# gasparian/CRNN-OCR-lite

Hardware: AMD Instinct MI355X
Metric: text-line images/sec (train step) (higher is better)
Workload: dtype bf16; 1 GPU; BASELINE configs[1]: 100x32x1 text lines, batch 256/GPU, max_len 23, time_dense_size 128, n_units 256 BiLSTM, STN on, dropout on, CTC, Adam(1e-4,b1=.5,clipnorm 5), bf16 MFMA products, bf16 conv-stack tensors in HBM, fp32 accumulate/statistics/RNN/optimizer (outside the 1e-3 parity tolerance: see parity_mode for the fp32 step); global_batch=256, parallelism=dp1, parity_mode_backward_planes=2 (16 significant bits per factor; CRNN_FLAG_THREE_PLANE_BACKWARD = strict)

## Files before the change

crnn-ocr-lite_amd/crnn_mi355x/native.py:

```python
import ctypes
import os
import re
import subprocess

HERE = os.path.dirname(os.path.abspath(__file__))
PKG_ROOT = os.path.dirname(HERE)
REPO_ROOT = os.path.dirname(PKG_ROOT)
HEADER = os.path.join(REPO_ROOT, "include", "crnn_mi355x.h")
CSRC = os.path.join(PKG_ROOT, "csrc")
LIB_PATH = os.path.join(PKG_ROOT, "libcrnn_mi355x.so")
HOOKS_HEADER = os.path.join(REPO_ROOT, "include", "crnn_testhooks.h")
HOOKS_PATH = os.path.join(PKG_ROOT, "libcrnn_testhooks.so")
SOURCES = ["gemm.hip", "gemm_nt.hip", "gemm_wres.hip", "gemm_wres3.hip", "gemm_wgrad.hip", "gemm_wgrad3.hip", "gemm_pres.hip", "conv.hip", "conv_bwd_fused.hip", "dwconv_stream.hip", "dwconv_bwd_stream.hip", "stn.hip", "rnn.hip", "rnn_persist.hip", "gru_persist.hip", "ctc.hip", "dense.hip", "beam.hip", "score.hip", "optim.hip", "ingest.hip", "model.hip"]


class crnn_config(ctypes.Structure):
    _fields_ = [(n, ctypes.c_int) for n in
                ("batch", "imgh", "imgw", "num_classes", "max_len", "tds", "units", "gru", "stn", "dropout", "mfma_bf16", "flags")]


FLAG_RNN_STEP_KERNELS = 1
FLAG_GEMM_TILE_KERNELS = 2
FLAG_NO_DW_BN_FUSION = 8
FLAG_NO_DW_BWD_FUSION = 16
FLAG_DW_TILE_KERNEL = 32
FLAG_RNN_LINEAR_CLUSTERS = 64
FLAG_NO_BN_STATS_FUSION = 128
FLAG_F32_MFMA_GEMMS = 256
FLAG_BN2_DW_FUSION = 1024
FLAG_BN2_STATS_FUSION = 2048
FLAG_BLOCK1_KERNELS = 16384
FLAG_LOC_NET_KERNELS = 8192
FLAG_THREE_PLANE_BACKWARD = 65536
FLAG_TWO_PLANE_FORWARD = 131072
FLAG_NO_GRADIENT_PLANES = 262144
FLAG_NO_POOL_ARGMAX_Q = 524288
FLAG_NO_BN2_DW_FUSION = 4096
RNN_XCD_LOCAL = 0x100


_CTYPE = [("crnn_stream_t", ctypes.c_void_p), ("size_t", ctypes.c_size_t), ("uint64_t", ctypes.c_uint64),
          ("uint32_t", ctypes.c_uint32), ("long", ctypes.c_long), ("int", ctypes.c_int), ("float", ctypes.c_float),
          ("double", ctypes.c_double)]


def _ctype_of(decl):
    decl = decl.strip()
    if "*" in decl:
        return ctypes.c_void_p
    for key, ct in _CTYPE:
        if re.search(r"\b%s\b" % key, decl):
# ... 91 lines not shown
```

crnn-ocr-lite_amd/csrc/conv.hip:

```cpp
#include "common.h"
#include <stdlib.h>

#define BN_EPS 1e-3f
#ifndef DW_NT
#define DW_NT 256
#endif

template <int VEC>
struct VecF { float v[VEC]; };

#ifndef CRNN_NT_BN_BWD2
#define CRNN_NT_BN_BWD2 1
#endif
#ifndef CRNN_NT_BN_ACT
#define CRNN_NT_BN_ACT 1
#endif
template <int VEC, typename T>
__device__ __forceinline__ VecF<VEC> vload_nt(const T* p);
template <int VEC, bool NT, typename T>
__device__ __forceinline__ VecF<VEC> vload_s(const T* p);
template <int VEC, typename T>
__device__ __forceinline__ VecF<VEC> vload(const T* p) {
  VecF<VEC> r;
  if (VEC == 8) {
// ... 2 lines not shown
    r.v[4 % VEC] = q.hi.x; r.v[5 % VEC] = q.hi.y; r.v[6 % VEC] = q.hi.z; r.v[7 % VEC] = q.hi.w;
  } else if (VEC == 4) {
    float4 q = ld4(p); r.v[0] = q.x; r.v[1 % VEC] = q.y; r.v[2 % VEC] = q.z; r.v[3 % VEC] = q.w;
  } else {
    r.v[0] = ld1(p);
  }
  return r;
}
template <int VEC, typename T>
__device__ __forceinline__ void vstore(T* p, const VecF<VEC>& r) {
  if (VEC == 8) {
    float8 q;
    q.lo = make_float4(r.v[0], r.v[1 % VEC], r.v[2 % VEC], r.v[3 % VEC]);
    q.hi = make_float4(r.v[4 % VEC], r.v[5 % VEC], r.v[6 % VEC], r.v[7 % VEC]);
    st8(p, q);
  } else if (VEC == 4) {
    st4(p, make_float4(r.v[0], r.v[1 % VEC], r.v[2 % VEC], r.v[3 % VEC]));
  } else {
    st1(p, r.v[0]);
  }
}
template <typename T> struct VecMax { static const int value = 4; };
template <> struct VecMax<bf16_t> { static const int value = 8; };

#ifndef DW_BF16_VN
#define DW_BF16_VN 4
#endif
template <typename T> struct RawV;
template <> struct RawV<float> { typedef float4 type; static const int N = 4; };
#if DW_BF16_VN == 8
template <> struct RawV<bf16_t> { typedef uint4 type; static const int N = 8; };
#else
template <> struct RawV<bf16_t> { typedef uint2 type; static const int N = 4; };
#endif
template <typename V, typename T> __device__ __forceinline__ V ldraw(const T* p) { return *reinterpret_cast<const V*>(p); }
__device__ __forceinline__ void widen(const float4& v, float (&f)[4]) { f[0] = v.x; f[1] = v.y; f[2] = v.z; f[3] = v.w; }
__device__ __forceinline__ void widen(const uint2& u, float (&f)[4]) {
  f[0] = __uint_as_float(u.x << 16); f[1] = __uint_as_float(u.x & 0xffff0000u);
  f[2] = __uint_as_float(u.y << 16); f[3] = __uint_as_float(u.y & 0xffff0000u);
}
__device__ __forceinline__ void widen(const uint4& u, float (&f)[8]) {
  f[0] = __uint_as_float(u.x << 16); f[1] = __uint_as_float(u.x & 0xffff0000u);
  f[2] = __uint_as_float(u.y << 16); f[3] = __uint_as_float(u.y & 0xffff0000u);
  f[4] = __uint_as_float(u.z << 16); f[5] = __uint_as_float(u.z & 0xffff0000u);
  f[6] = __uint_as_float(u.w << 16); f[7] = __uint_as_float(u.w & 0xffff0000u);
}
// ... 696 lines not shown
  if (dt_in == CRNN_BF16) return bn_act_launch((const bf16_t*)x, bnstate, (float*)y, B, H, W, C, ph, pw, rate, seed, layer, stream);
  if (dt_out == CRNN_BF16) return bn_act_launch((const float*)x, bnstate, (bf16_t*)y, B, H, W, C, ph, pw, rate, seed, layer, stream);
  return bn_act_launch((const float*)x, bnstate, (float*)y, B, H, W, C, ph, pw, rate, seed, layer, stream);
}
extern "C" int crnn_bn_act_pool_drop_qmax_ex(const void* x, const float* bnstate, void* y, void* qmax, int B, int H, int W, int C, int ph, int pw, float rate,
                                             uint64_t seed, uint32_t layer, int dt_in, int dt_out, hipStream_t stream) {
  if (!x || !bnstate || !qmax) return CRNN_ERR_ARG;
  if (dt_in == CRNN_BF16 && dt_out == CRNN_BF16) return bn_act_launch((const bf16_t*)x, bnstate, (bf16_t*)y, B, H, W, C, ph, pw, rate, seed, layer, stream, (bf16_t*)qmax);
  if (dt_in == CRNN_BF16) return bn_act_launch((const bf16_t*)x, bnstate, (float*)y, B, H, W, C, ph, pw, rate, seed, layer, stream, (bf16_t*)qmax);
  if (dt_out == CRNN_BF16) return bn_act_launch((const float*)x, bnstate, (bf16_t*)y, B, H, W, C, ph, pw, rate, seed, layer, stream, (float*)qmax);
  return bn_act_launch((const float*)x, bnstate, (float*)y, B, H, W, C, ph, pw, rate, seed, layer, stream, (float*)qmax);
}
extern "C" int crnn_bn_act_pool_drop(const float* x, const float* bnstate, float* y, int B, int H, int W, int C, int ph,
                                     int pw, float rate, uint64_t seed, uint32_t layer, hipStream_t stream) {
  return crnn_bn_act_pool_drop_ex(x, bnstate, y, B, H, W, C, ph, pw, rate, seed, layer, CRNN_F32, CRNN_F32, stream);
}

template <typename T>
struct BnBwdArgsT {
  const T* x; const T* g; const float* bnstate; const float* gamma;
  int B, H, W, C, ph, pw; float rate; uint64_t seed; uint32_t layer;
  unsigned short* dxp = nullptr; long dxps = 0; int dxpl = 0;
  const T* qmax = nullptr;
};
template <int VEC, typename T>
__device__ __forceinline__ void bn_store_dx(const BnBwdArgsT<T>& a, T* dx, long idx, const VecF<VEC>& o) {
  if constexpr (VEC == 4 && sizeof(T) == 4) {
    if (a.dxp) {
      unsigned w0[3], w1[3];
      crnn_split3_pair(o.v[0], o.v[1], w0[0], w0[1], w0[2]);
      crnn_split3_pair(o.v[2 % VEC], o.v[3 % VEC], w1[0], w1[1], w1[2]);
      unsigned short* q = a.dxp + idx;
      *reinterpret_cast<uint2*>(q) = make_uint2(w0[0], w1[0]);
      *reinterpret_cast<uint2*>(q + a.dxps) = make_uint2(w0[1], w1[1]);
      if (a.dxpl == 3) *reinterpret_cast<uint2*>(q + 2 * a.dxps) = make_uint2(w0[2], w1[2]);
      return;
    }
  }
  vstore<VEC>(&dx[idx], o);
}

template <int VEC, typename T>
__device__ __forceinline__ VecF<VEC> vload_nt(const T* p) {
  typedef unsigned u32x4_nt __attribute__((ext_vector_type(4)));
  VecF<VEC> r;
  if constexpr (VEC == 8 && sizeof(T) == 2) {
    const u32x4_nt u = __builtin_nontemporal_load(reinterpret_cast<const u32x4_nt*>(p));
// ... 42 lines not shown
      for (int j = 0; j < a.pw; ++j) {
        if (ii == si && j == sj) continue;
        VecF<VEC> o = vload_s<VEC, NT>(&a.x[(((long)b * a.H + ho * a.ph + ii) * a.W + wo * a.pw + j) * a.C + c0]);
        bool earlier = (ii < si) || (ii == si && j < sj);
#pragma unroll
        for (int e = 0; e < VEC; ++e) {
          float oy = relu6f(fmaf(o.v[e], sc.v[e], sh.v[e]));
          if (earlier ? (oy >= y.v[e]) : (oy > y.v[e])) arg[e] = false;
        }
      }
    oidx = (((long)b * Ho + ho) * Wo + wo) * a.C + c0;
  }
  VecF<VEC> gv = vload_s<VEC, NT>(&a.g[oidx]);
  float dm[VEC];
  drop_scale_vec<VEC>(a.seed, a.layer, (uint64_t)oidx, a.rate, inv_keep, dm);
#pragma unroll
  for (int e = 0; e < VEC; ++e) {
    bool live = arg[e] && (y.v[e] > 0.f) && (y.v[e] < 6.f);
    out.v[e] = live ? gv.v[e] * dm[e] : 0.f;
  }
  return out;
}

template <int PASS, int VEC, bool POOL, typename T>
__global__ __launch_bounds__(256) void bn_bwd_kernel(BnBwdArgsT<T> a, float* __restrict__ partials,
                                                     const float* __restrict__ coef, T* __restrict__ dx, int CW,
                                                     int rows_per_chunk) {
  __shared__ float red[2][256 * VEC];
  const int tid = threadIdx.x, cl = tid % CW, rt = tid / CW, RT = 256 / CW;
  const long M = (long)a.B * a.H * a.W;
  const long r0 = (long)blockIdx.x * rows_per_chunk;
  long r1 = r0 + rows_per_chunk; if (r1 > M) r1 = M;
  const int CL = a.C / VEC;
  const float inv_keep = a.rate > 0.f ? 1.f / (1.f - a.rate) : 1.f;
  for (int cb = 0; cb < CL; cb += CW) {
    const int c = cb + cl, c0 = c * VEC;
    VecF<VEC> s, q;
#pragma unroll
    for (int e = 0; e < VEC; ++e) { s.v[e] = 0.f; q.v[e] = 0.f; }
    if (c < CL) {
      VecF<VEC> mu = vload<VEC>(a.bnstate + c0), var = vload<VEC>(a.bnstate + a.C + c0);
      VecF<VEC> sc = vload<VEC>(a.bnstate + 2 * a.C + c0), sh = vload<VEC>(a.bnstate + 3 * a.C + c0);
      VecF<VEC> inv, c1, c2;
#pragma unroll
      for (int e = 0; e < VEC; ++e) { inv.v[e] = 1.0f / sqrtf(var.v[e] + BN_EPS); c1.v[e] = 0.f; c2.v[e] = 0.f; }
      VecF<VEC> Pc, Qc;
#pragma unroll
      for (int e = 0; e < VEC; ++e) { Pc.v[e] = 0.f; Qc.v[e] = 0.f; }
      if (PASS == 2) {
        c1 = vload<VEC>(coef + c0); c2 = vload<VEC>(coef + a.C + c0);
#pragma unroll
        for (int e = 0; e < VEC; ++e) bn_bwd_pq(sc.v[e], c1.v[e], c2.v[e], mu.v[e], inv.v[e], Pc.v[e], Qc.v[e]);
      }
      long r = r0 + rt;
#if CRNN_BNB_ROWS4
      if (PASS == 1 && !POOL) {
        for (; r + 3L * RT < r1; r += 4L * RT) {
          VecF<VEC> xr[4], gr[4];
#pragma unroll
          for (int u = 0; u < 4; ++u) xr[u] = vload<VEC>(&a.x[(r + u * RT) * a.C + c0]);
#pragma unroll
          for (int u = 0; u < 4; ++u) gr[u] = bn_gy_vec<VEC, POOL, T>(a, r + u * RT, c0, xr[u], sc, sh, inv_keep);
#pragma unroll
          for (int u = 0; u < 4; ++u)
#pragma unroll
            for (int e = 0; e < VEC; ++e) { s.v[e] += gr[u].v[e]; q.v[e] = fmaf(gr[u].v[e], (xr[u].v[e] - mu.v[e]) * inv.v[e], q.v[e]); }
        }
      }
#endif
      constexpr bool NT = CRNN_NT_BN_BWD2 && PASS == 2;
      for (; r + RT < r1; r += 2L * RT) {
        VecF<VEC> xa = vload_s<VEC, NT>(&a.x[r * a.C + c0]);
        VecF<VEC> xb = vload_s<VEC, NT>(&a.x[(r + RT) * a.C + c0]);
        VecF<VEC> ga = bn_gy_vec<VEC, POOL, T, NT>(a, r, c0, xa, sc, sh, inv_keep);
        VecF<VEC> gb = bn_gy_vec<VEC, POOL, T, NT>(a, r + RT, c0, xb, sc, sh, inv_keep);
        VecF<VEC> oa, ob;
#pragma unroll
        for (int e = 0; e < VEC; ++e) {
          float ha = (xa.v[e] - mu.v[e]) * inv.v[e], hb = (xb.v[e] - mu.v[e]) * inv.v[e];
          if (PASS == 1) {
            s.v[e] += ga.v[e]; q.v[e] = fmaf(ga.v[e], ha, q.v[e]);
            s.v[e] += gb.v[e]; q.v[e] = fmaf(gb.v[e], hb, q.v[e]);
          } else {
            oa.v[e] = bn_bwd_dx_pq(xa.v[e], ga.v[e], sc.v[e], Pc.v[e], Qc.v[e]);
            ob.v[e] = bn_bwd_dx_pq(xb.v[e], gb.v[e], sc.v[e], Pc.v[e], Qc.v[e]);
          }
        }
        if (PASS == 2) { bn_store_dx<VEC, T>(a, dx, r * a.C + c0, oa); bn_store_dx<VEC, T>(a, dx, (r + RT) * a.C + c0, ob); }
      }
      for (; r < r1; r += RT) {
        VecF<VEC> xv = vload_s<VEC, NT>(&a.x[r * a.C + c0]);
        VecF<VEC> gy = bn_gy_vec<VEC, POOL, T, NT>(a, r, c0, xv, sc, sh, inv_keep);
        VecF<VEC> o;
#pragma unroll
        for (int e = 0; e < VEC; ++e) {
          float xh = (xv.v[e] - mu.v[e]) * inv.v[e];
          if (PASS == 1) { s.v[e] += gy.v[e]; q.v[e] = fmaf(gy.v[e], xh, q.v[e]); }
          else o.v[e] = bn_bwd_dx_pq(xv.v[e], gy.v[e], sc.v[e], Pc.v[e], Qc.v[e]);
        }
        if (PASS == 2) bn_store_dx<VEC, T>(a, dx, r * a.C + c0, o);
      }
    }
    if (PASS == 1) {
      __syncthreads();
#pragma unroll
      for (int e = 0; e < VEC; ++e) { red[0][tid * VEC + e] = s.v[e]; red[1][tid * VEC + e] = q.v[e]; }
      __syncthreads();
      if (rt == 0 && c < CL) {
#pragma unroll
        for (int e = 0; e < VEC; ++e) {
          float s2 = 0.f, q2 = 0.f;
          for (int r = 0; r < RT; ++r) { s2 += red[0][(r * CW + cl) * VEC + e]; q2 += red[1][(r * CW + cl) * VEC + e]; }
          partials[((long)blockIdx.x * 2 + 0) * a.C + c0 + e] = s2;
          partials[((long)blockIdx.x * 2 + 1) * a.C + c0 + e] = q2;
// ... 771 lines not shown
  return CRNN_OK;
}
extern "C" int crnn_dwconv_c1_bwd_rows(int B, int H, int W) { return cdiv((long)B * H * W, 1024); }
extern "C" int crnn_dwconv3x3_c1_bwd(const float* d, const float* da, const float* bnstate, const float* coef, const float* x, const float* k, float* dx, float* dk,
                                     float* scratch, int B, int H, int W, hipStream_t stream) {
  if (!d || !da || !bnstate || !coef || !x || !k || !dk || !scratch || B <= 0 || H <= 0 || W <= 0) return CRNN_ERR_ARG;
  if ((long)B * H * W >= (1L << 31) || W > C1B_MAXW) return CRNN_ERR_UNSUPPORTED;
  const int rows = crnn_dwconv_c1_bwd_rows(B, H, W);
  hipLaunchKernelGGL(dwconv_c1_bwd_kernel, dim3(rows), dim3(256), 0, stream, d, da, bnstate, coef, x, k, dx, scratch, B, H, W);
  CRNN_LAUNCH_CHECK();
  return crnn_partials_sum(scratch, rows, 9, dk, 1.f, stream);
}
extern "C" int crnn_pw1_bn_bwd_rows(long M) { return cdiv(M, colreduce_rpc(M)); }
extern "C" int crnn_pw1_bn_bwd(const float* d, const float* in_bnstate, const float* w, const void* dq, float* da, float* dw, float* scratch,
                               float* bn_stat_partials, long M, int N, int dt_q, hipStream_t stream) {
  if (!d || !in_bnstate || !w || !dq || !da || !dw || !scratch || !bn_stat_partials) return CRNN_ERR_ARG;
  if (!pw1_ok(N, dq) || M <= 0 || N < 8) return CRNN_ERR_UNSUPPORTED;
  const int rpc = colreduce_rpc(M), chunks = cdiv(M, rpc);
  if (dt_q == CRNN_BF16) hipLaunchKernelGGL(pw1_bn_bwd_kernel<bf16_t>, dim3(chunks), dim3(256), 0, stream, d, in_bnstate, w, (const bf16_t*)dq, da, scratch, bn_stat_partials, M, N, rpc);
  else hipLaunchKernelGGL(pw1_bn_bwd_kernel<float>, dim3(chunks), dim3(256), 0, stream, d, in_bnstate, w, (const float*)dq, da, scratch, bn_stat_partials, M, N, rpc);
  CRNN_LAUNCH_CHECK();
  return crnn_partials_sum(scratch, chunks, N, dw, 1.f, stream);
}
```

crnn-ocr-lite_amd/csrc/model.hip:

```cpp
#include "common.h"
#include "crnn_mi355x.h"
#include <string.h>
#include <stdio.h>
#include <string>
#include <vector>

namespace {

struct BlockSpec { int cout, ph, pw; };
const BlockSpec kBlocks[7] = {{64, 1, 1}, {128, 1, 1}, {256, 2, 2}, {256, 1, 1}, {512, 1, 2}, {512, 1, 1}, {512, 1, 1}};
bool pool_argmax_q(const crnn_config* cfg, int block) {
  const int ph = kBlocks[block - 1].ph, pw = kBlocks[block - 1].pw;
  return !(cfg->flags & CRNN_FLAG_NO_POOL_ARGMAX_Q) && ((ph == 2 && pw == 2) || (ph == 1 && pw == 2));
}
const float kDropBlock = 0.1f, kDropDense1 = 0.4f, kDropRnn = 0.2f;
const uint32_t kLayerDense1 = 8, kLayerRnn = 9;

struct Tensor { std::string name; long off; long size; int ndim; int dims[4]; int dtype = CRNN_F32; };

struct Dims {
  int B, H0, W0, Hp, Wp, T, feat, C, L, tds, u, G, stn_flat;
  int Hs1, Ws1, Ho1, Wo1, Hs2, Ws2, Ho2, Wo2;
  int bh[8], bw[8], bc[8];
};
// ... 275 lines not shown
  return ((((uintptr_t)a) | ((uintptr_t)b) | ((uintptr_t)c) | ((uintptr_t)d)) & 15) == 0;
}
bool fuse_bn2_dw_shape(const crnn_config* cfg, const Dims& d, const Plan& P, int i) {
  if (i < 1 || i > 6) return false;
  if (!bn2_dw_fusion_block(cfg, i) || (cfg->flags & (CRNN_FLAG_DW_TILE_KERNEL | CRNN_FLAG_NO_DW_BWD_FUSION))) return false;
  const std::string p = std::to_string(i), n = std::to_string(i + 1);
  const bool pooled = kBlocks[i - 1].ph * kBlocks[i - 1].pw != 1;
  if (pooled && (!pool_argmax_q(cfg, i) || !P.has("qm" + p) || d.bh[i] % kBlocks[i - 1].ph || d.bw[i] % kBlocks[i - 1].pw || d.bc[i] % 4 ||
                 (long)d.B * d.bh[i + 1] * d.bw[i + 1] * d.bc[i] + 8192L * 256 * 8 >= (1L << 31))) return false;
  const int dt = P.dt("q" + p);
  if (P.dt("x" + p) != dt || P.dt("d" + n) != dt || P.off("dm" + p) < 0) return false;
  if (bn2_stats_fusion_block(cfg, i) && P.off("bn2parts") < 0) return false;
  const int H = d.bh[i + 1], W = d.bw[i + 1], C = d.bc[i];
  return crnn_dwconv_fwd_stream_pro_supported_ex(d.B, H, W, C, dt) == CRNN_OK && crnn_dwconv_bwd_stream_pro_supported_ex(d.B, H, W, C, dt) == CRNN_OK &&
         (dt == CRNN_F32 || crnn_dwconv_bwd_fused_supported(H, W, C) == CRNN_OK);
}
float* pro_src(const Ctx& c, int i) { return c.w((kBlocks[i - 1].ph * kBlocks[i - 1].pw != 1 ? "qm" : "q") + std::to_string(i)); }
bool fuse_bn2_dw(const Ctx& c, int i) {
  if (!fuse_bn2_dw_shape(c.cfg, c.d, c.P, i)) return false;
  const std::string p = std::to_string(i), n = std::to_string(i + 1);
  return aligned16(c.w("q" + p), c.w("bn2s" + p), c.w("d" + n), c.p("b" + n + "_dw")) && aligned16(pro_src(c, i));
}
const float* keep_bytes(const Ctx& c, int i) { return c.cfg->dropout ? c.w("dm" + std::to_string(i)) : nullptr; }
int gemm32(const Ctx& c, int mode, const float* A, const float* B, float* C, int M, int N, int K, int lda, int ldb, int ldc,
           const float* bias = nullptr, int act = 0, int acc = 0, int perm = 0) {
  return crnn_gemm_f32(mode, A, B, C, M, N, K, lda, ldb, ldc, bias, act, acc, perm, c.scratch(), kGemmScratchBytes, c.s);
}

int colsum(const Ctx& c, const float* x, long M, int C, int ld, float* out) {
  CRNN_TRY(crnn_colreduce(x, c.partials(), M, C, ld, 1, c.s));
  return crnn_partials_sum(c.partials(), crnn_colreduce_chunks(M), C, out, 1.f, c.s);
}

int check_cfg(const crnn_config* c) {
  if (!c || c->batch <= 0) return CRNN_ERR_ARG;
  if (c->units < 64 || c->units % 64) return CRNN_ERR_UNSUPPORTED;
  if (c->mfma_bf16 < 0 || c->mfma_bf16 > 2) return CRNN_ERR_ARG;
  if (c->num_classes > 64 || c->num_classes < 2) return CRNN_ERR_UNSUPPORTED;
  if (2 * c->max_len + 1 > 64) return CRNN_ERR_UNSUPPORTED;
  if (c->tds % 4) return CRNN_ERR_UNSUPPORTED;
  Dims d = make_dims(c);
  if (c->stn && (d.Ho2 < 1 || d.Wo2 < 1)) return CRNN_ERR_UNSUPPORTED;
  if (d.T < 3 || d.feat < 1) return CRNN_ERR_UNSUPPORTED;
  return 0;
}

// ... 280 lines not shown
          rc = conv_planes(cfg, false) == 2 ? crnn_pwconv_bnrelu6_fwd_f32x2(dd, s1, c.p(bp + "_pw"), qq, M, co, ci, parts, stream)
                                            : crnn_pwconv_bnrelu6_fwd_f32x3(dd, s1, c.p(bp + "_pw"), qq, M, co, ci, parts, stream);
        CRNN_TRY(rc);
      }
      else if (fuse_a) {
        int rc = CRNN_ERR_UNSUPPORTED;
        if (wt && dtq == CRNN_BF16 && !(cfg->flags & CRNN_FLAG_GEMM_TILE_KERNELS) && crnn_pwconv_fwd_wres_supported(M, co, ci) == CRNN_OK) {
          rc = crnn_pwconv_bnrelu6_fwd_wres(dd, s1, wq, qq, M, co, ci, parts, stream);
          if (rc == CRNN_OK) stat_rows = crnn_pwconv_fwd_wres_rows(M, co, ci);
        }
        if (rc == CRNN_ERR_UNSUPPORTED) rc = crnn_pwconv_bnrelu6_fwd(dd, s1, wq, qq, M, co, ci, parts, dtq, wt, stream);
        CRNN_TRY(rc);
      } else CRNN_TRY(crnn_pwconv_fwd(aa, wq, qq, M, co, ci, parts, nullptr, pw_products_fwd(cfg),
                                      dtd, dtw, dtq, wt, stream));
    }
    CRNN_TRY(crnn_bn_finalize_folded(parts, stat_rows, co, M, c.p(bp + "_bn2_g"), c.p(bp + "_bn2_b"), s2, c.w("fold"), stream));
    bn_off += co;
    if (fuse_bn2_dw(c, i)) {
      if (ph * pw != 1)
        CRNN_TRY(crnn_bn_act_pool_drop_qmax_ex(qq, s2, nullptr, pro_src(c, i), B, H, W, co, ph, pw, 0.f, seed, (uint32_t)i, dtq, dtq, stream));
      pro_q = pro_src(c, i); pro_s2 = s2; in = nullptr;
      continue;
    }
    if (use_qmax(c, i))
      CRNN_TRY(crnn_bn_act_pool_drop_qmax_ex(qq, s2, xo, c.w("qm" + p), B, H, W, co, ph, pw, cfg->dropout ? kDropBlock : 0.f, seed, (uint32_t)i, dtq, c.dt("x" + p), stream));
    else
    CRNN_TRY(crnn_bn_act_pool_drop_ex(qq, s2, xo, B, H, W, co, ph, pw, cfg->dropout ? kDropBlock : 0.f, seed,
                                      (uint32_t)i, dtq, c.dt("x" + p), stream));
    in = xo;
  }
  if (keep_pending) { CRNN_TRY(fj.join()); keep_pending = false; }
  const int T = d.T, TB = T * B, u = d.u, G = d.G;
  int rc1 = CRNN_ERR_UNSUPPORTED;
  if (d1T_off >= 0 && c.dt("x7") == CRNN_BF16)
    rc1 = crnn_dense_fwd_stream(in, reinterpret_cast<const bf16_t*>(c.w("pwT")) + d1T_off, c.p("dense1_b"), c.w("dn1"), TB, d.tds, d.feat, d.feat, d.feat, 1, T,
                                (train && cfg->dropout) ? kDropDense1 : 0.f, seed, kLayerDense1, stream);
  if (rc1 != CRNN_OK && rc1 != CRNN_ERR_UNSUPPORTED) return rc1;
  if (rc1 != CRNN_OK) {
    CRNN_TRY(gemm_t(c, 0, in, c.dt("x7"), c.p("dense1_w"), CRNN_F32, c.w("dn1"), CRNN_F32, TB, d.tds, d.feat, d.feat, d.tds, d.tds, c.p("dense1_b"), 1, 0, T));
    if (train && cfg->dropout) CRNN_TRY(crnn_dropout(c.w("dn1"), c.w("dn1"), TB, d.tds, d.tds, d.tds, kDropDense1, seed, kLayerDense1, stream));
  }
  const int dtu = rnn_dtu(cfg);
  const bool persist = rnn_persist(cfg);
  const size_t xbytes = persist ? crnn_lstm_persist_xbuf_bytes(T, B, u, dtu) : 0;
  const bool xw_stream = dtu == CRNN_BF16 && !(cfg->flags & CRNN_FLAG_GEMM_TILE_KERNELS) && TB % 64 == 0 && G % 128 == 0 && d.tds % 64 == 0 && u % 64 == 0;
  {
    long in_off[8], out_off[8]; int R[8], Cc[8]; int n = 0;
// ... 292 lines not shown
  float* gA = c.w("gA"); float* gB = c.w("gB"); float* gC = c.w("gC");
  hipEvent_t gB_free = nullptr, gC_free = nullptr;
  int bn2_stats_rows = 0;
  for (int i = 7; i >= 1; --i) {
    std::string p = std::to_string(i), bp = "b" + p;
    const int H = d.bh[i], W = d.bw[i], ci = d.bc[i - 1], co = d.bc[i];
    const long M = (long)B * H * W;
    const int dtd = c.dt("d" + p), dtq = c.dt("q" + p);
    const bool fused_bf = i > 1 && dtd == CRNN_BF16 && c.dt("x" + std::to_string(i - 1)) == CRNN_BF16 && !(cfg->flags & CRNN_FLAG_NO_DW_BWD_FUSION) &&
                          crnn_dwconv_bwd_fused_supported(H, W, ci) == CRNN_OK;
    const bool fused_f32 = i > 1 && dtd == CRNN_F32 && dtq == CRNN_F32 && c.dt("x" + std::to_string(i - 1)) == CRNN_F32 &&
                           !(cfg->flags & (CRNN_FLAG_NO_DW_BWD_FUSION | CRNN_FLAG_DW_TILE_KERNEL)) &&
                           crnn_dwconv_bwd_stream_supported_ex(B, H, W, ci, CRNN_F32) == CRNN_OK &&
                           aligned16(c.w("d" + p), c.w("x" + std::to_string(i - 1)), c.p(bp + "_dw"), c.w("coef")) && aligned16(gA, gB, gC, c.w("bn1s" + p));
    const bool fused_dw = fused_bf || fused_f32;
    int bn1_stats_rows = 0;
    const bool dq_planes = !fused_bf && pw_products(cfg) == 2 && conv_planes(cfg, true) == 2 && dtq == CRNN_F32 && dtd == CRNN_F32 && fuse_dw_bn_x3(cfg, dtd, dtq, ci) &&
                           !(cfg->flags & (CRNN_FLAG_GEMM_TILE_KERNELS | CRNN_FLAG_NO_BN_STATS_FUSION | CRNN_FLAG_NO_GRADIENT_PLANES)) &&
                           (kBlocks[i - 1].ph * kBlocks[i - 1].pw == 1 || crnn_knob("CRNN_DQPL_POOL", 1)) &&
                           crnn_gemm_pres_supported(M, ci, co, 2) == CRNN_OK && crnn_pwconv_wgrad_planes_stream_supported(M, co, ci) == CRNN_OK &&
                           crnn_pwconv_wgrad_planes_stream_scratch_bytes(M, co, ci) <= kGemmScratchBytes &&
                           aligned16(c.w("d" + p), c.w("q" + p), c.w("bn1s" + p), c.p(bp + "_pw")) && aligned16(gA, gB, gC, c.w("partials"));
    CRNN_TRY(fj.wait(gB_free)); gB_free = nullptr;
    if (bn2_stats_rows > 0) {
      CRNN_TRY(crnn_bn_bwd_finalize(c.w("bn2parts"), bn2_stats_rows, co, M, c.g(bp + "_bn2_g"), c.g(bp + "_bn2_b"), c.w("coef"), stream));
      if (dq_planes)
        CRNN_TRY(crnn_bn_bwd_apply_planes_ex(c.w("q" + p), gA, c.w("bn2s" + p), c.w("coef"), gB, M * co, 2, B, H, W, co, kBlocks[i - 1].ph, kBlocks[i - 1].pw,
                                             cfg->dropout ? kDropBlock : 0.f, seed, (uint32_t)i, stream));
      else
      CRNN_TRY(crnn_bn_bwd_apply_ex(c.w("q" + p), gA, c.w("bn2s" + p), c.w("coef"), gB, B, H, W, co, kBlocks[i - 1].ph, kBlocks[i - 1].pw,
                                    cfg->dropout ? kDropBlock : 0.f, seed, (uint32_t)i, dtq, stream));
      bn2_stats_rows = 0;
    } else if (use_qmax(c, i))
      CRNN_TRY(crnn_bn_bwd_qmax_ex(c.w("q" + p), c.w("qm" + p), gA, c.w("bn2s" + p), c.p(bp + "_bn2_g"), dq_planes ? nullptr : gB, dq_planes ? gB : nullptr, M * co,
                                   dq_planes ? 2 : 0, c.g(bp + "_bn2_g"), c.g(bp + "_bn2_b"), c.w("partials"), c.w("coef"), B, H, W, co, kBlocks[i - 1].ph,
                                   kBlocks[i - 1].pw, cfg->dropout ? kDropBlock : 0.f, seed, (uint32_t)i, dtq, stream));
    else if (dq_planes)
      CRNN_TRY(crnn_bn_bwd_planes_ex(c.w("q" + p), gA, c.w("bn2s" + p), c.p(bp + "_bn2_g"), gB, M * co, 2, c.g(bp + "_bn2_g"), c.g(bp + "_bn2_b"), c.w("partials"),
                                     c.w("coef"), B, H, W, co, kBlocks[i - 1].ph, kBlocks[i - 1].pw, cfg->dropout ? kDropBlock : 0.f, seed, (uint32_t)i, stream));
    else
    CRNN_TRY(crnn_bn_bwd_ex(c.w("q" + p), gA, c.w("bn2s" + p), c.p(bp + "_bn2_g"), gB, c.g(bp + "_bn2_g"), c.g(bp + "_bn2_b"), c.w("partials"),
                            c.w("coef"), B, H, W, co, kBlocks[i - 1].ph, kBlocks[i - 1].pw, cfg->dropout ? kDropBlock : 0.f, seed, (uint32_t)i, dtq, stream));
    if (block1_fused(cfg, ci, dtd)) {
      const int rows = crnn_pw1_bn_bwd_rows(M);
      float* bnp = c.w("partials");
      CRNN_TRY(crnn_pw1_bn_bwd(c.w("d" + p), c.w("bn1s" + p), c.p(bp + "_pw"), gB, gA, c.g(bp + "_pw"), bnp + ((2L * rows + 63) & ~63L), bnp, M, co, dtq, stream));
      bn1_stats_rows = rows;
    } else if (ci == 1 && dtd == CRNN_F32) {
      CRNN_TRY(crnn_pw1_bwd(c.w("a" + p), c.p(bp + "_pw"), gB, gA, c.g(bp + "_pw"), c.w("partials"), M, co, dtq, stream));
    } else {
      const bool side = fj.on && fused_dw;
      const Ctx& cw = side ? ca : c;
      if (side) CRNN_TRY(fj.fork());
      if (fuse_dw_bn(cfg, dtd, dtq, ci)) {
        int rc = CRNN_ERR_UNSUPPORTED;
        if (!(cfg->flags & CRNN_FLAG_GEMM_TILE_KERNELS) && crnn_pwconv_wgrad_stream_supported(M, co, ci) == CRNN_OK)
          rc = crnn_pwconv_bnrelu6_wgrad_stream(c.w("d" + p), c.w("bn1s" + p), gB, c.g(bp + "_pw"), M, co, ci, cw.scratch(), kGemmScratchBytes, cw.s);
        if (rc == CRNN_ERR_UNSUPPORTED)
          rc = crnn_pwconv_bnrelu6_wgrad(c.w("d" + p), c.w("bn1s" + p), gB, c.g(bp + "_pw"), M, co, ci, cw.scratch(), kGemmScratchBytes, cw.s);
        CRNN_TRY(rc);
      }
      else if (fuse_dw_bn_x3(cfg, dtd, dtq, ci) && aligned16(c.w("d" + p), c.w("q" + p), c.w("bn1s" + p), c.p(bp + "_pw"))) {
        int rc = CRNN_ERR_UNSUPPORTED;
        if (dq_planes) { CRNN_TRY(crnn_pwconv_bnrelu6_wgrad_planes_stream_gp(c.w("d" + p), c.w("bn1s" + p), gB, M * co, c.g(bp + "_pw"), M, co, ci, cw.scratch(), kGemmScratchBytes, cw.s)); rc = CRNN_OK; }
        if (rc == CRNN_ERR_UNSUPPORTED)
          rc = (conv_planes(cfg, true) == 2 ? crnn_pwconv_bnrelu6_wgrad_f32x2 : crnn_pwconv_bnrelu6_wgrad_f32x3)(
              c.w("d" + p), c.w("bn1s" + p), gB, c.g(bp + "_pw"), M, co, ci, cw.scratch(), kGemmScratchBytes, cw.s);
        CRNN_TRY(rc);
// ... 150 lines not shown
```

include/crnn_mi355x.h:

```cpp
#ifndef CRNN_MI355X_H
#define CRNN_MI355X_H
#include <stddef.h>
#include <stdint.h>
#ifdef __cplusplus
extern "C" {
#endif

typedef struct ihipStream_t* crnn_stream_t;

typedef struct {
  int batch;
  int imgh, imgw;
  int num_classes;
  int max_len;
  int tds;
  int units;
  int gru;
  int stn;
  int dropout;
  int mfma_bf16;
  int flags;
} crnn_config;
#define CRNN_FLAG_BLOCK1_KERNELS 16384
#define CRNN_FLAG_LOC_NET_KERNELS 8192
#define CRNN_FLAG_NO_BN2_DW_FUSION 4096
#define CRNN_FLAG_BN2_STATS_FUSION 2048
#define CRNN_FLAG_BN2_DW_FUSION 1024
#define CRNN_FLAG_DW_TILE_KERNEL 32
#define CRNN_FLAG_NO_DW_BWD_FUSION 16
#define CRNN_FLAG_NO_DW_BN_FUSION 8
#define CRNN_FLAG_GEMM_TILE_KERNELS 2
#define CRNN_FLAG_THREE_PLANE_BACKWARD 65536
#define CRNN_FLAG_TWO_PLANE_FORWARD 131072
#define CRNN_FLAG_NO_GRADIENT_PLANES 262144
#define CRNN_FLAG_NO_POOL_ARGMAX_Q 524288
#define CRNN_FLAG_F32_MFMA_GEMMS 256
#define CRNN_FLAG_NO_BN_STATS_FUSION 128
#define CRNN_FLAG_RNN_LINEAR_CLUSTERS 64
#define CRNN_FLAG_RNN_STEP_KERNELS 1

int  crnn_num_params(const crnn_config* cfg);
long crnn_params_total(const crnn_config* cfg);
int  crnn_param_info(const crnn_config* cfg, int idx, char* name, int name_cap, long* offset, long* size,
                     int* ndim, int* dims );
int  crnn_bn_total(const crnn_config* cfg);
int  crnn_bn_info(const crnn_config* cfg, int idx, char* name, int name_cap, int* offset, int* channels, long* count);
int  crnn_time_steps(const crnn_config* cfg);

size_t crnn_workspace_bytes(const crnn_config* cfg);
int  crnn_ws_tensor(const crnn_config* cfg, const char* name, long* offset, long* count);
int  crnn_block_output_fused(const crnn_config* cfg, int block);
int  crnn_ws_tensor_info(const crnn_config* cfg, const char* name, long* offset, long* count, int* dtype);


int crnn_forward(const crnn_config* cfg, const float* params, const float* bn_mean, const float* bn_var,
                 const float* x, float* ws, size_t ws_bytes, float* y_pred, int train, uint64_t seed,
                 crnn_stream_t stream);
int crnn_forward_ex(const crnn_config* cfg, const float* params, const float* bn_mean, const float* bn_var,
// ... 85 lines not shown
int crnn_pwconv_bnrelu6_wgrad_planes_stream_gp(const float* d, const float* in_bnstate, const void* g_planes, long g_plane_stride, float* dw, long M, int N, int K,
                                               float* scratch, size_t scratch_bytes, crnn_stream_t stream);
int crnn_gemm_tn_planes_stream(const float* A, int lda, const float* B, int ldb, float* C, int ldc, int M, int N, long K, float* scratch,
                               size_t scratch_bytes, crnn_stream_t stream);
int crnn_gemm_nt_f32x2_stream(const float* A0, const float* W0, const float* A1, const float* W1, float* Y, int M, int N, int K, int lda, int ldw, int ldy,
                              crnn_stream_t stream);
int crnn_gemm_pres_supported(long M, int N, int K, int planes);
int crnn_gemm_pres_stat_rows(long M, int N, int K, int planes);
int crnn_gemm_pres_bnstats(const void* dq_planes, long plane_stride, const float* w, float* da, long M, int N, int K, int planes, const float* d,
                           const float* bnstate, float* stat_partials, void* a_planes, long a_stride, int a_count, crnn_stream_t stream);
int crnn_pw1_fwd(const float* a, const float* w, void* q, long M, int N, float* stat_partials, int dt_q, crnn_stream_t stream);
int crnn_pw1_fwd_folded(const float* a, const float* w, void* y, long M, int N, const float* out_bnstate, int dt_y, crnn_stream_t stream);
int crnn_pw1_bwd(const float* a, const float* w, const void* dq, float* da, float* dw, float* scratch, long M, int N, int dt_q,
                 crnn_stream_t stream);
int crnn_dwconv_c1_stat_rows(int B, int H, int W);
int crnn_dwconv3x3_c1_fwd(const float* x, const float* k, float* out, float* stat_partials, int B, int H, int W, crnn_stream_t stream);
int crnn_pw1_bn_fwd(const float* d, const float* in_bnstate, const float* w, void* q, long M, int N, float* stat_partials, int dt_q, crnn_stream_t stream);
int crnn_dwconv_c1_bwd_rows(int B, int H, int W);
int crnn_dwconv3x3_c1_bwd(const float* d, const float* da, const float* bnstate, const float* coef, const float* x, const float* k, float* dx, float* dk,
                          float* scratch, int B, int H, int W, crnn_stream_t stream);
int crnn_pw1_bn_bwd_rows(long M);
int crnn_pw1_bn_bwd(const float* d, const float* in_bnstate, const float* w, const void* dq, float* da, float* dw, float* scratch, float* bn_stat_partials,
                    long M, int N, int dt_q, crnn_stream_t stream);
int crnn_dwconv3x3_bn_relu6_fwd(const void* x, const float* k, const float* bnstate, void* out, int B, int H, int W, int C,
                                int dtype, crnn_stream_t stream);
int crnn_dwconv_fwd_stream_supported(int B, int H, int W, int C);
int crnn_dwconv_fwd_stream_rows(int B, int H, int W, int C);
int crnn_dwconv3x3_fwd_stream(const void* x, const float* k, void* out, float* stat_partials, const float* bnstate, int B, int H, int W, int C,
                              int flip, crnn_stream_t stream);
int crnn_dwconv3x3_fwd_stream_ex(const void* x, const float* k, void* out, float* stat_partials, const float* bnstate, int B, int H, int W, int C,
                                 int flip, int out_order, crnn_stream_t stream);
int crnn_dwconv_fwd_stream_pro_supported(int B, int H, int W, int C);
int crnn_dwconv3x3_fwd_stream_pro(const void* q, const float* pro_bnstate, float rate, const void* keep, const float* k, void* out,
                                  float* stat_partials, int B, int H, int W, int C, crnn_stream_t stream);
int crnn_transpose_batch(const float* src, void* dst, int n, const long* in_off, const long* out_off, const int* R, const int* C,
                         int dt_out, crnn_stream_t stream);
int crnn_dwconv3x3_fwd_ex(const void* x, const float* k, void* out, float* stat_partials, int B, int H, int W, int C, int flip,
                          int dtype, crnn_stream_t stream);
int crnn_dwconv3x3_wgrad_ex(const void* x, const void* g, float* dk, float* scratch, int B, int H, int W, int C, int dtype,
                            crnn_stream_t stream);
int crnn_colreduce_ex(const void* x, float* partials, long M, int C, int ld, int nv, int dtype, crnn_stream_t stream);
int crnn_bn_act_pool_drop_ex(const void* x, const float* bnstate, void* y, int B, int H, int W, int C, int ph, int pw, float rate,
                             uint64_t seed, uint32_t layer, int dt_in, int dt_out, crnn_stream_t stream);
int crnn_bn_bwd_ex(const void* x, const void* g, const float* bnstate, const float* gamma, void* dx, float* dgamma, float* dbeta,
                   float* scratch_partials, float* coef, int B, int H, int W, int C, int ph, int pw, float rate, uint64_t seed,
                   uint32_t layer, int dtype, crnn_stream_t stream);
// ... 213 lines not shown
```

Baseline: 43640 images/sec.

## Recompute block-1 pointwise output from 1-channel input instead of reading q1

For block 1, whose pointwise conv has a single input channel, the pre-BN2 tensor q1 is rebuilt on the fly from the scalar per-pixel input d times the weight vector, with bf16 rounding. This happens in the forward BN/act/dropout kernel and in the backward BN-stats and dx passes. A new fused backward kernel combines the BN2 dx, pointwise weight gradient, data gradient and BN1 stats in one pass. The intent is to drop HBM reads of the wide q1 tensor in exchange for extra ALU work and new kernel paths gated by alignment and dtype checks.

```diff
diff --git a/crnn-ocr-lite_amd/crnn_mi355x/native.py b/crnn-ocr-lite_amd/crnn_mi355x/native.py
--- a/crnn-ocr-lite_amd/crnn_mi355x/native.py
+++ b/crnn-ocr-lite_amd/crnn_mi355x/native.py
@@ -27,6 +27,7 @@
 FLAG_RNN_LINEAR_CLUSTERS = 64
 FLAG_NO_BN_STATS_FUSION = 128
 FLAG_F32_MFMA_GEMMS = 256
+FLAG_BLOCK1_READS_Q1 = 512
 FLAG_BN2_DW_FUSION = 1024
 FLAG_BN2_STATS_FUSION = 2048
 FLAG_BLOCK1_KERNELS = 16384
diff --git a/crnn-ocr-lite_amd/csrc/conv.hip b/crnn-ocr-lite_amd/csrc/conv.hip
--- a/crnn-ocr-lite_amd/csrc/conv.hip
+++ b/crnn-ocr-lite_amd/csrc/conv.hip
@@ -48,6 +48,18 @@
 }
 template <typename T> struct VecMax { static const int value = 4; };
 template <> struct VecMax<bf16_t> { static const int value = 8; };
+__device__ __forceinline__ float q1_act(float dv, float sc1, float sh1) { return relu6f(fmaf(dv, sc1, sh1)); }
+template <int VEC>
+__device__ __forceinline__ VecF<VEC> q1_form(float av, const VecF<VEC>& wv) {
+  static_assert(VEC % 2 == 0, "q1_form rounds in pairs");
+  VecF<VEC> o;
+#pragma unroll
+  for (int e = 0; e < VEC; e += 2) {
+    const unsigned u = pack2_bf16(av * wv.v[e], av * wv.v[e + 1]);
+    o.v[e] = __uint_as_float(u << 16); o.v[e + 1] = __uint_as_float(u & 0xffff0000u);
+  }
+  return o;
+}
 
 #ifndef DW_BF16_VN
 #define DW_BF16_VN 4
@@ -790,7 +802,13 @@
   int B, H, W, C, ph, pw; float rate; uint64_t seed; uint32_t layer;
   unsigned short* dxp = nullptr; long dxps = 0; int dxpl = 0;
   const T* qmax = nullptr;
+  const float* q1d = nullptr; const float* q1bn = nullptr; const float* q1w = nullptr;
 };
+template <int VEC, bool NT, bool VQ1, typename T>
+__device__ __forceinline__ VecF<VEC> bn_x_vec(const BnBwdArgsT<T>& a, long r, int c0, const VecF<VEC>& wq, float sc1, float sh1) {
+  if constexpr (VQ1) return q1_form<VEC>(q1_act(a.q1d[r], sc1, sh1), wq);
+  else return vload_s<VEC, NT>(&a.x[r * a.C + c0]);
+}
 template <int VEC, typename T>
 __device__ __forceinline__ void bn_store_dx(const BnBwdArgsT<T>& a, T* dx, long idx, const VecF<VEC>& o) {
   if constexpr (VEC == 4 && sizeof(T) == 4) {
@@ -879,7 +897,7 @@
   return out;
 }
 
-template <int PASS, int VEC, bool POOL, typename T>
+template <int PASS, int VEC, bool POOL, typename T, bool VQ1 = false>
 __global__ __launch_bounds__(256) void bn_bwd_kernel(BnBwdArgsT<T> a, float* __restrict__ partials,
                                                      const float* __restrict__ coef, T* __restrict__ dx, int CW,
                                                      int rows_per_chunk) {
@@ -904,6 +922,10 @@
       VecF<VEC> Pc, Qc;
 #pragma unroll
       for (int e = 0; e < VEC; ++e) { Pc.v[e] = 0.f; Qc.v[e] = 0.f; }
+      VecF<VEC> wq; float sc1 = 0.f, sh1 = 0.f;
+#pragma unroll
+      for (int e = 0; e < VEC; ++e) wq.v[e] = 0.f;
+      if constexpr (VQ1) { wq = vload<VEC>(a.q1w + c0); sc1 = a.q1bn[2]; sh1 = a.q1bn[3]; }
       if (PASS == 2) {
         c1 = vload<VEC>(coef + c0); c2 = vload<VEC>(coef + a.C + c0);
 #pragma unroll
@@ -915,7 +937,7 @@
         for (; r + 3L * RT < r1; r += 4L * RT) {
           VecF<VEC> xr[4], gr[4];
 #pragma unroll
-          for (int u = 0; u < 4; ++u) xr[u] = vload<VEC>(&a.x[(r + u * RT) * a.C + c0]);
+          for (int u = 0; u < 4; ++u) xr[u] = bn_x_vec<VEC, false, VQ1, T>(a, r + u * RT, c0, wq, sc1, sh1);
 #pragma unroll
           for (int u = 0; u < 4; ++u) gr[u] = bn_gy_vec<VEC, POOL, T>(a, r + u * RT, c0, xr[u], sc, sh, inv_keep);
 #pragma unroll
@@ -927,8 +949,8 @@
 #endif
       constexpr bool NT = CRNN_NT_BN_BWD2 && PASS == 2;
       for (; r + RT < r1; r += 2L * RT) {
-        VecF<VEC> xa = vload_s<VEC, NT>(&a.x[r * a.C + c0]);
-        VecF<VEC> xb = vload_s<VEC, NT>(&a.x[(r + RT) * a.C + c0]);
+        VecF<VEC> xa = bn_x_vec<VEC, NT, VQ1, T>(a, r, c0, wq, sc1, sh1);
+        VecF<VEC> xb = bn_x_vec<VEC, NT, VQ1, T>(a, r + RT, c0, wq, sc1, sh1);
         VecF<VEC> ga = bn_gy_vec<VEC, POOL, T, NT>(a, r, c0, xa, sc, sh, inv_keep);
         VecF<VEC> gb = bn_gy_vec<VEC, POOL, T, NT>(a, r + RT, c0, xb, sc, sh, inv_keep);
         VecF<VEC> oa, ob;
@@ -946,7 +968,7 @@
         if (PASS == 2) { bn_store_dx<VEC, T>(a, dx, r * a.C + c0, oa); bn_store_dx<VEC, T>(a, dx, (r + RT) * a.C + c0, ob); }
       }
       for (; r < r1; r += RT) {
-        VecF<VEC> xv = vload_s<VEC, NT>(&a.x[r * a.C + c0]);
+        VecF<VEC> xv = bn_x_vec<VEC, NT, VQ1, T>(a, r, c0, wq, sc1, sh1);
         VecF<VEC> gy = bn_gy_vec<VEC, POOL, T, NT>(a, r, c0, xv, sc, sh, inv_keep);
         VecF<VEC> o;
 #pragma unroll
@@ -1764,3 +1786,124 @@
   CRNN_LAUNCH_CHECK();
   return crnn_partials_sum(scratch, chunks, N, dw, 1.f, stream);
 }
+
+__global__ __launch_bounds__(256) void bn_act_drop_q1_kernel(const float* __restrict__ d, const float* __restrict__ bn1, const float* __restrict__ w,
+                                                             const float* __restrict__ bnstate, bf16_t* __restrict__ y, unsigned total, int C, float rate,
+                                                             uint64_t seed, uint32_t layer) {
+  const unsigned CL = (unsigned)C / 8;
+  const float inv_keep = rate > 0.f ? 1.f / (1.f - rate) : 1.f;
+  const float sc1 = bn1[2], sh1 = bn1[3];
+  const unsigned i0 = blockIdx.x * blockDim.x + threadIdx.x;
+  const int c0 = (int)(i0 % CL) * 8;
+  const VecF<8> s = vload<8>(bnstate + 2 * C + c0), t = vload<8>(bnstate + 3 * C + c0), wv = vload<8>(w + c0);
+  for (unsigned i = i0; i < total; i += gridDim.x * blockDim.x) {
+    const unsigned pix = i / CL;
+    const VecF<8> v = q1_form<8>(q1_act(d[pix], sc1, sh1), wv);
+    VecF<8> m;
+#pragma unroll
+    for (int e = 0; e < 8; ++e) m.v[e] = relu6f(fmaf(v.v[e], s.v[e], t.v[e]));
+    const long obase = (long)pix * C + c0;
+    float dm[8];
+    drop_scale_vec<8>(seed, layer, (uint64_t)obase, rate, inv_keep, dm);
+#pragma unroll
+    for (int e = 0; e < 8; ++e) m.v[e] *= dm[e];
+    vstore<8>(&y[obase], m);
+  }
+}
+__global__ __launch_bounds__(256) void pw1_bn2_bwd_kernel(BnBwdArgsT<bf16_t> a, const float* __restrict__ coef, float* __restrict__ da,
+                                                          float* __restrict__ partials, float* __restrict__ bnparts, long M, int rows_per_chunk) {
+  __shared__ float red[256 * 8];
+  __shared__ float sred[2][256];
+  const int N = a.C, CG = N / 8, RT = 256 / CG, tid = threadIdx.x, cg = tid % CG, rt = tid / CG, c0 = 8 * cg;
+  const long r0 = (long)blockIdx.x * rows_per_chunk;
+  long r1 = r0 + rows_per_chunk; if (r1 > M) r1 = M;
+  const float mu = a.q1bn[0], inv = 1.0f / sqrtf(a.q1bn[1] + BN_EPS), sc = a.q1bn[2], sh = a.q1bn[3];
+  const float inv_keep = a.rate > 0.f ? 1.f / (1.f - a.rate) : 1.f;
+  const VecF<8> wl = vload<8>(a.q1w + c0);
+  const VecF<8> sc2 = vload<8>(a.bnstate + 2 * N + c0), sh2 = vload<8>(a.bnstate + 3 * N + c0);
+  VecF<8> Pc, Qc;
+  {
+    const VecF<8> mu2 = vload<8>(a.bnstate + c0), var2 = vload<8>(a.bnstate + N + c0), c1 = vload<8>(coef + c0), c2 = vload<8>(coef + N + c0);
+#pragma unroll
+    for (int e = 0; e < 8; ++e) bn_bwd_pq(sc2.v[e], c1.v[e], c2.v[e], mu2.v[e], 1.0f / sqrtf(var2.v[e] + BN_EPS), Pc.v[e], Qc.v[e]);
+  }
+  float s[8], sg = 0.f, sq = 0.f;
+#pragma unroll
+  for (int e = 0; e < 8; ++e) s[e] = 0.f;
+  if (rt < RT)
+    for (long r = r0 + rt; r < r1; r += RT) {
+      const float dv = a.q1d[r], t = fmaf(dv, sc, sh), av = relu6f(t);
+      const VecF<8> xv = q1_form<8>(av, wl);
+      const VecF<8> gy = bn_gy_vec<8, false, bf16_t, (CRNN_NT_BN_BWD2 != 0)>(a, r, c0, xv, sc2, sh2, inv_keep);
+      VecF<8> g;
+#pragma unroll
+      for (int e = 0; e < 8; e += 2) {
+        const unsigned u = pack2_bf16(bn_bwd_dx_pq(xv.v[e], gy.v[e], sc2.v[e], Pc.v[e], Qc.v[e]), bn_bwd_dx_pq(xv.v[e + 1], gy.v[e + 1], sc2.v[e + 1], Pc.v[e + 1], Qc.v[e + 1]));
+        g.v[e] = __uint_as_float(u << 16); g.v[e + 1] = __uint_as_float(u & 0xffff0000u);
+      }
+      float acc = 0.f;
+#pragma unroll
+      for (int e = 0; e < 8; ++e) { s[e] = fmaf(av, g.v[e], s[e]); acc = fmaf(g.v[e], wl.v[e], acc); }
+      for (int o = 1; o < CG; o <<= 1) acc += __shfl_xor(acc, o, 64);
+      if (cg == 0) {
+        da[r] = acc;
+        const float gy1 = (t > 0.f && t < 6.f) ? acc : 0.f;
+        sg += gy1; sq = fmaf(gy1, (dv - mu) * inv, sq);
+      }
+    }
+#pragma unroll
+  for (int e = 0; e < 8; ++e) red[tid * 8 + e] = s[e];
+  sred[0][tid] = sg; sred[1][tid] = sq;
+  __syncthreads();
+  if (tid < N) {
+    float acc = 0.f;
+    for (int r = 0; r < RT; ++r) acc += red[(r * CG + tid / 8) * 8 + (tid & 7)];
+    partials[(long)blockIdx.x * N + tid] = acc;
+  }
+  if (tid < 2) {
+    float acc = 0.f;
+    for (int r = 0; r < RT; ++r) acc += sred[tid][r * CG];
+    bnparts[(long)blockIdx.x * 2 + tid] = acc;
+  }
+}
+extern "C" int crnn_block1_q1_supported(long M, int N) {
+  return (M > 0 && N >= 8 && N <= 256 && (N & (N - 1)) == 0 && M * N + 8192L * 256 * 8 < (1L << 31)) ? CRNN_OK : CRNN_ERR_UNSUPPORTED;
+}
+static bool q1_aligned(const void* a, const void* b, const void* c, const void* d, const void* e = nullptr, const void* f = nullptr) {
+  return ((((uintptr_t)a | (uintptr_t)b | (uintptr_t)c | (uintptr_t)d | (uintptr_t)e | (uintptr_t)f) & 15) == 0);
+}
+extern "C" int crnn_bn_act_drop_q1(const float* d, const float* in_bnstate, const float* w, const float* out_bnstate, void* x, long M, int N, float rate,
+                                   uint64_t seed, uint32_t layer, hipStream_t stream) {
+  if (!d || !in_bnstate || !w || !out_bnstate || !x) return CRNN_ERR_ARG;
+  if (crnn_block1_q1_supported(M, N) != CRNN_OK || !q1_aligned(w, out_bnstate, x, nullptr)) return CRNN_ERR_UNSUPPORTED;
+  const long total = M * (N / 8);
+  int blocks = cdiv(total, 256); if (blocks > 8192) blocks = 8192;
+  hipLaunchKernelGGL(bn_act_drop_q1_kernel, dim3(blocks), dim3(256), 0, stream, d, in_bnstate, w, out_bnstate, (bf16_t*)x, (unsigned)total, N, rate, seed, layer);
+  CRNN_LAUNCH_CHECK();
+  return CRNN_OK;
+}
+extern "C" int crnn_bn_bwd_stats_q1(const float* d, const float* in_bnstate, const float* w, const void* g, const float* out_bnstate, float* dgamma, float* dbeta,
+                                    float* scratch_partials, float* coef, long M, int N, float rate, uint64_t seed, uint32_t layer, hipStream_t stream) {
+  if (!d || !in_bnstate || !w || !g || !out_bnstate || !dgamma || !dbeta || !scratch_partials || !coef) return CRNN_ERR_ARG;
+  if (crnn_block1_q1_supported(M, N) != CRNN_OK || !q1_aligned(w, g, out_bnstate, coef)) return CRNN_ERR_UNSUPPORTED;
+  BnBwdArgsT<bf16_t> a{nullptr, (const bf16_t*)g, out_bnstate, nullptr, 1, 1, (int)M, N, 1, 1, rate, seed, layer};
+  a.q1d = d; a.q1bn = in_bnstate; a.q1w = w;
+  const int CL = N / 8, CW = pow2_ge(CL < 256 ? CL : 256);
+  const int rpc = bn_bwd_rows_per_chunk(M), chunks = cdiv(M, rpc);
+  hipLaunchKernelGGL((bn_bwd_kernel<1, 8, false, bf16_t, true>), dim3(chunks), dim3(256), 0, stream, a, scratch_partials, (const float*)nullptr, (bf16_t*)nullptr, CW, rpc);
+  CRNN_LAUNCH_CHECK();
+  hipLaunchKernelGGL(bn_bwd_finalize_kernel, dim3(cdiv(N, RED_CH)), dim3(RED_CH, RED_PL), 0, stream, scratch_partials, chunks, N, 1.0 / (double)M, dgamma, dbeta, coef);
+  CRNN_LAUNCH_CHECK();
+  return CRNN_OK;
+}
+extern "C" int crnn_pw1_bn2_bwd(const float* d, const float* in_bnstate, const float* w, const void* g, const float* out_bnstate, const float* coef, float* da,
+                                float* dw, float* scratch, float* bn_stat_partials, long M, int N, float rate, uint64_t seed, uint32_t layer, hipStream_t stream) {
+  if (!d || !in_bnstate || !w || !g || !out_bnstate || !coef || !da || !dw || !scratch || !bn_stat_partials) return CRNN_ERR_ARG;
+  if (crnn_block1_q1_supported(M, N) != CRNN_OK || !q1_aligned(w, g, out_bnstate, coef)) return CRNN_ERR_UNSUPPORTED;
+  BnBwdArgsT<bf16_t> a{nullptr, (const bf16_t*)g, out_bnstate, nullptr, 1, 1, (int)M, N, 1, 1, rate, seed, layer};
+  a.q1d = d; a.q1bn = in_bnstate; a.q1w = w;
+  const int rpc = colreduce_rpc(M), chunks = cdiv(M, rpc);
+  hipLaunchKernelGGL(pw1_bn2_bwd_kernel, dim3(chunks), dim3(256), 0, stream, a, coef, da, scratch, bn_stat_partials, M, rpc);
+  CRNN_LAUNCH_CHECK();
+  return crnn_partials_sum(scratch, chunks, N, dw, 1.f, stream);
+}
diff --git a/crnn-ocr-lite_amd/csrc/model.hip b/crnn-ocr-lite_amd/csrc/model.hip
--- a/crnn-ocr-lite_amd/csrc/model.hip
+++ b/crnn-ocr-lite_amd/csrc/model.hip
@@ -321,6 +321,13 @@
   return aligned16(c.w("q" + p), c.w("bn2s" + p), c.w("d" + n), c.p("b" + n + "_dw")) && aligned16(pro_src(c, i));
 }
 const float* keep_bytes(const Ctx& c, int i) { return c.cfg->dropout ? c.w("dm" + std::to_string(i)) : nullptr; }
+bool block1_q1_formed(const Ctx& c) {
+  const crnn_config* cfg = c.cfg; const Dims& d = c.d;
+  if ((cfg->flags & CRNN_FLAG_BLOCK1_READS_Q1) || !block1_fused(cfg, d.bc[0], c.dt("d1")) || kBlocks[0].ph * kBlocks[0].pw != 1) return false;
+  if (c.dt("q1") != CRNN_BF16 || c.dt("x1") != CRNN_BF16 || c.gdt() != CRNN_BF16 || fuse_bn2_dw(c, 1)) return false;
+  return crnn_block1_q1_supported((long)d.B * d.bh[1] * d.bw[1], d.bc[1]) == CRNN_OK && aligned16(c.p("b1_pw"), c.w("x1"), c.w("bn2s1"), c.w("coef")) &&
+         aligned16(c.w("gA"), c.w("gB"), c.w("gC"));
+}
 int gemm32(const Ctx& c, int mode, const float* A, const float* B, float* C, int M, int N, int K, int lda, int ldb, int ldc,
            const float* bias = nullptr, int act = 0, int acc = 0, int perm = 0) {
   return crnn_gemm_f32(mode, A, B, C, M, N, K, lda, ldb, ldc, bias, act, acc, perm, c.scratch(), kGemmScratchBytes, c.s);
@@ -647,7 +654,9 @@
       pro_q = pro_src(c, i); pro_s2 = s2; in = nullptr;
       continue;
     }
-    if (use_qmax(c, i))
+    if (i == 1 && block1_q1_formed(c))
+      CRNN_TRY(crnn_bn_act_drop_q1(dd, s1, c.p(bp + "_pw"), s2, xo, M, co, cfg->dropout ? kDropBlock : 0.f, seed, (uint32_t)i, stream));
+    else if (use_qmax(c, i))
       CRNN_TRY(crnn_bn_act_pool_drop_qmax_ex(qq, s2, xo, c.w("qm" + p), B, H, W, co, ph, pw, cfg->dropout ? kDropBlock : 0.f, seed, (uint32_t)i, dtq, c.dt("x" + p), stream));
     else
     CRNN_TRY(crnn_bn_act_pool_drop_ex(qq, s2, xo, B, H, W, co, ph, pw, cfg->dropout ? kDropBlock : 0.f, seed,
@@ -986,6 +995,7 @@
                            crnn_pwconv_wgrad_planes_stream_scratch_bytes(M, co, ci) <= kGemmScratchBytes &&
                            aligned16(c.w("d" + p), c.w("q" + p), c.w("bn1s" + p), c.p(bp + "_pw")) && aligned16(gA, gB, gC, c.w("partials"));
     CRNN_TRY(fj.wait(gB_free)); gB_free = nullptr;
+    const bool q1_formed = i == 1 && bn2_stats_rows == 0 && block1_q1_formed(c);
     if (bn2_stats_rows > 0) {
       CRNN_TRY(crnn_bn_bwd_finalize(c.w("bn2parts"), bn2_stats_rows, co, M, c.g(bp + "_bn2_g"), c.g(bp + "_bn2_b"), c.w("coef"), stream));
       if (dq_planes)
@@ -995,7 +1005,10 @@
       CRNN_TRY(crnn_bn_bwd_apply_ex(c.w("q" + p), gA, c.w("bn2s" + p), c.w("coef"), gB, B, H, W, co, kBlocks[i - 1].ph, kBlocks[i - 1].pw,
                                     cfg->dropout ? kDropBlock : 0.f, seed, (uint32_t)i, dtq, stream));
       bn2_stats_rows = 0;
-    } else if (use_qmax(c, i))
+    } else if (q1_formed)
+      CRNN_TRY(crnn_bn_bwd_stats_q1(c.w("d" + p), c.w("bn1s" + p), c.p(bp + "_pw"), gA, c.w("bn2s" + p), c.g(bp + "_bn2_g"), c.g(bp + "_bn2_b"), c.w("partials"),
+                                    c.w("coef"), M, co, cfg->dropout ? kDropBlock : 0.f, seed, (uint32_t)i, stream));
+    else if (use_qmax(c, i))
       CRNN_TRY(crnn_bn_bwd_qmax_ex(c.w("q" + p), c.w("qm" + p), gA, c.w("bn2s" + p), c.p(bp + "_bn2_g"), dq_planes ? nullptr : gB, dq_planes ? gB : nullptr, M * co,
                                    dq_planes ? 2 : 0, c.g(bp + "_bn2_g"), c.g(bp + "_bn2_b"), c.w("partials"), c.w("coef"), B, H, W, co, kBlocks[i - 1].ph,
                                    kBlocks[i - 1].pw, cfg->dropout ? kDropBlock : 0.f, seed, (uint32_t)i, dtq, stream));
@@ -1008,6 +1021,11 @@
     if (block1_fused(cfg, ci, dtd)) {
       const int rows = crnn_pw1_bn_bwd_rows(M);
       float* bnp = c.w("partials");
+      if (q1_formed) {
+        CRNN_TRY(crnn_pw1_bn2_bwd(c.w("d" + p), c.w("bn1s" + p), c.p(bp + "_pw"), gA, c.w("bn2s" + p), c.w("coef"), gB, c.g(bp + "_pw"), bnp + ((2L * rows + 63) & ~63L), bnp,
+                                  M, co, cfg->dropout ? kDropBlock : 0.f, seed, (uint32_t)i, stream));
+        float* t = gA; gA = gB; gB = t;
+      } else
       CRNN_TRY(crnn_pw1_bn_bwd(c.w("d" + p), c.w("bn1s" + p), c.p(bp + "_pw"), gB, gA, c.g(bp + "_pw"), bnp + ((2L * rows + 63) & ~63L), bnp, M, co, dtq, stream));
       bn1_stats_rows = rows;
     } else if (ci == 1 && dtd == CRNN_F32) {
diff --git a/include/crnn_mi355x.h b/include/crnn_mi355x.h
--- a/include/crnn_mi355x.h
+++ b/include/crnn_mi355x.h
@@ -34,6 +34,7 @@
 #define CRNN_FLAG_TWO_PLANE_FORWARD 131072
 #define CRNN_FLAG_NO_GRADIENT_PLANES 262144
 #define CRNN_FLAG_NO_POOL_ARGMAX_Q 524288
+#define CRNN_FLAG_BLOCK1_READS_Q1 512
 #define CRNN_FLAG_F32_MFMA_GEMMS 256
 #define CRNN_FLAG_NO_BN_STATS_FUSION 128
 #define CRNN_FLAG_RNN_LINEAR_CLUSTERS 64
@@ -165,6 +166,13 @@
 int crnn_pw1_bn_bwd_rows(long M);
 int crnn_pw1_bn_bwd(const float* d, const float* in_bnstate, const float* w, const void* dq, float* da, float* dw, float* scratch, float* bn_stat_partials,
                     long M, int N, int dt_q, crnn_stream_t stream);
+int crnn_block1_q1_supported(long M, int N);
+int crnn_bn_act_drop_q1(const float* d, const float* in_bnstate, const float* w, const float* out_bnstate, void* x, long M, int N, float rate, uint64_t seed,
+                        uint32_t layer, crnn_stream_t stream);
+int crnn_bn_bwd_stats_q1(const float* d, const float* in_bnstate, const float* w, const void* g, const float* out_bnstate, float* dgamma, float* dbeta,
+                         float* scratch_partials, float* coef, long M, int N, float rate, uint64_t seed, uint32_t layer, crnn_stream_t stream);
+int crnn_pw1_bn2_bwd(const float* d, const float* in_bnstate, const float* w, const void* g, const float* out_bnstate, const float* coef, float* da, float* dw,
+                     float* scratch, float* bn_stat_partials, long M, int N, float rate, uint64_t seed, uint32_t layer, crnn_stream_t stream);
 int crnn_dwconv3x3_bn_relu6_fwd(const void* x, const float* k, const float* bnstate, void* out, int B, int H, int W, int C,
                                 int dtype, crnn_stream_t stream);
 int crnn_dwconv_fwd_stream_supported(int B, int H, int W, int C);
```

After: 43570 images/sec. No clear change (-0.2%).
